# Murmeldyret/cubesat-APDS

Measured on AMD Instinct MI355X. Metric: frames/sec (detect+match+homography) 4k×4k tile vs 1M-desc DB; Mmatches/sec, higher is better.
Workload: dtype fp4 e2m1 operands / f32 accumulate = exact integer Hamming (match), f32 (AKAZE), f64 (homography solve)

## Files before the change

### cubesat-apds_amd/csrc/hamming_mfma.hip

```cpp
#include <atomic>
#include <memory>

#include "config.h"
#include "kernels.h"

namespace apds {

typedef int hm_v8i __attribute__((ext_vector_type(8)));
typedef float hm_f32x4 __attribute__((ext_vector_type(4)));

#ifndef APDS_HM_WAVES
#define APDS_HM_WAVES 8
#endif
static constexpr int HM_WAVES = APDS_HM_WAVES;
static constexpr int HM_TM = 16 * HM_WAVES;
#ifndef APDS_HM_WPE
#define APDS_HM_WPE 4
#endif
#ifndef APDS_HM_NC
#define APDS_HM_NC 3
#endif
static constexpr int HM_NC = APDS_HM_NC;
static constexpr int HM_Q = HM_WAVES * 16 * HM_NC;
static constexpr int HM_UNIT_SCALE = 0x7F7F7F7F;
static constexpr uint64_t HM_EMPTY = ~0ull;
static constexpr int HM_BIAS = 1024;

__device__ __forceinline__ uint32_t hm_spread8(uint32_t b, uint32_t nib) {
    uint32_t t = b & 0xFFu;
    t = (t | (t << 12)) & 0x000F000Fu;
    t = (t | (t << 6)) & 0x03030303u;
    t = (t | (t << 3)) & 0x11111111u;
    return t * nib;
}

__global__ __launch_bounds__(256) void hm_expand_rows_kernel(const uint32_t* __restrict__ rows, long long n, uint32_t nib, int bias, uint4* __restrict__ out,
                                                             float* __restrict__ pc) {
    APDS_RAISE_WAVE_PRIORITY();
    const long long i = (long long)blockIdx.x * 256 + threadIdx.x;
    const uint32_t d = i < n * 16 ? rows[i] : 0u;
    int v = __popc(d);
#pragma unroll
    for (int off = 8; off > 0; off >>= 1) v += __shfl_xor(v, off);
    if (i >= n * 16) return;
    out[i] = make_uint4(hm_spread8(d, nib), hm_spread8(d >> 8, nib), hm_spread8(d >> 16, nib), hm_spread8(d >> 24, nib));
    if ((threadIdx.x & 15) == 0) pc[i >> 4] = (float)(v + bias);
}

__global__ void hm_pad_rows_kernel(uint4* __restrict__ rows, float* __restrict__ pc, long long n, long long n_pad) {
    const long long i = n + (threadIdx.x >> 4);
    if (i >= n_pad) return;
    for (long long r = i; r < n_pad; r += 8) {
        rows[r * 16 + (threadIdx.x & 15)] = make_uint4(0, 0, 0, 0);
        if ((threadIdx.x & 15) == 0) pc[r] = INFINITY;
    }
}

__global__ void hm_thresholds_kernel(const uint64_t* __restrict__ topk, int K, const float* __restrict__ qpc, int nq, uint32_t* __restrict__ thr) {
    const int i = blockIdx.x * blockDim.x + threadIdx.x;
    if (i >= nq) return;
    const uint64_t k2 = topk[(size_t)i * K + K - 1];
    thr[i] = k2 == HM_EMPTY ? 0x7F800000u : __float_as_uint((float)((int)(uint32_t)(k2 >> 32) - (int)qpc[i] + HM_BIAS));
}

struct HmTop2 {
    uint32_t d0, d1;
    uint32_t i0, i1;
};
__device__ __forceinline__ void hm_insert(HmTop2& b, uint32_t d, uint32_t idx) {
    if (d < b.d1) {
        if (d < b.d0) {
            b.d1 = b.d0;
            b.i1 = b.i0;
            b.d0 = d;
            b.i0 = idx;
        } else {
            b.d1 = d;
            b.i1 = idx;
        }
    }
}

template <int PRIO, bool THR>
__global__ __launch_bounds__(64 * HM_WAVES) __attribute__((amdgpu_waves_per_eu(APDS_HM_WPE, APDS_HM_WPE))) void hamming_mfma_kernel(const uint4* __restrict__ train_fp4, const float* __restrict__ tpc, int n_train,
                                                           const uint4* __restrict__ query_fp4, const float* __restrict__ qpc, int nq, int tiles_per_split,
                                                           int q_tiles, int splits, uint32_t index_base, const uint32_t* __restrict__ thr,
                                                           uint64_t* __restrict__ out) {
    extern __shared__ __attribute__((aligned(128))) unsigned char hm_lds[];
    constexpr int TILE_BYTES = HM_TM * 256;
    const int tid = threadIdx.x, lane = tid & 63, wave = tid >> 6;
    int split, qtile;
    if ((splits & 7) == 0) {
        const int xcd = blockIdx.x & 7, j = blockIdx.x >> 3;
        split = xcd + 8 * (j / q_tiles);
        qtile = j % q_tiles;
    } else {
        split = blockIdx.x / q_tiles;
        qtile = blockIdx.x % q_tiles;
    }
    const int q0 = qtile * HM_Q + wave * 16 * HM_NC;
    const int n_tiles = (n_train + HM_TM - 1) / HM_TM;
    const int tile_begin = split * tiles_per_split, tile_end = min(n_tiles, tile_begin + tiles_per_split);
    const int col = lane & 15, kq = lane >> 4;

    uint4 B[HM_NC][4];
    float qq[HM_NC];
#pragma unroll
    for (int c = 0; c < HM_NC; c++) {
        const int qi = min(q0 + 16 * c + col, nq - 1);
#pragma unroll
        for (int s = 0; s < 4; s++) B[c][s] = query_fp4[(size_t)qi * 16 + 4 * s + kq];
        qq[c] = qpc[qi];
    }
    HmTop2 best[HM_NC];
#pragma unroll
    for (int c = 0; c < HM_NC; c++) {
        best[c].d0 = best[c].d1 = THR ? thr[min(q0 + 16 * c + col, nq - 1)] : 0x7F800000u;
        best[c].i0 = best[c].i1 = 0xFFFFFFFFu;
    }

    if (tile_begin < tile_end) {
        int soff[4];
#pragma unroll
        for (int i = 0; i < 4; i++) {
            const int r = 16 * wave + 4 * i + (lane >> 4);
            soff[i] = r * 256 + (((lane & 15) ^ (r & 15)) << 4);
        }
        auto stage = [&](int tile, int buf) {
            const unsigned char* tbase = reinterpret_cast<const unsigned char*>(train_fp4) + (size_t)tile * TILE_BYTES;
#pragma unroll
            for (int i = 0; i < 4; i++)
                __builtin_amdgcn_global_load_lds((const __attribute__((address_space(1))) void*)(tbase + soff[i]),
                                                 (__attribute__((address_space(3))) void*)(hm_lds + buf * TILE_BYTES + (16 * wave + 4 * i) * 256), 16, 0, 0);
            if (wave < HM_TM / 64)
                __builtin_amdgcn_global_load_lds((const __attribute__((address_space(1))) void*)(tpc + (size_t)tile * HM_TM + 64 * wave + lane),
                                                 (__attribute__((address_space(3))) void*)(hm_lds + 2 * TILE_BYTES + buf * (HM_TM * 4) + 256 * wave), 4, 0, 0);
        };
        int aoff[4];
#pragma unroll
        for (int s = 0; s < 4; s++) aoff[s] = col * 256 + (((4 * s + kq) ^ col) << 4);
        const int noff = 2 * TILE_BYTES + 16 * kq;

        hm_f32x4 acc[HM_NC];
        auto rank = [&](const hm_f32x4 (&a)[HM_NC], uint32_t row0) {
            bool hit[HM_NC];
#pragma unroll
            for (int c = 0; c < HM_NC; c++) {
                const uint32_t mn = min(min(__float_as_uint(a[c][0]), __float_as_uint(a[c][1])), min(__float_as_uint(a[c][2]), __float_as_uint(a[c][3])));
                hit[c] = mn < best[c].d1;
            }
#pragma unroll
            for (int c = 0; c < HM_NC; c++)
                if (__any(hit[c])) {
#pragma unroll
                    for (int j = 0; j < 4; j++) hm_insert(best[c], __float_as_uint(a[c][j]), row0 + j);
                }
        };

        stage(tile_begin, 0);
        __syncthreads();
        for (int tile = tile_begin; tile < tile_end; tile++) {
            const int buf = (tile - tile_begin) & 1;
            if (tile + 1 < tile_end) stage(tile + 1, buf ^ 1);
            const unsigned char* T = hm_lds + buf * TILE_BYTES;
            const unsigned char* Nn = hm_lds + noff + buf * (HM_TM * 4);
#pragma unroll
            for (int rb = 0; rb < HM_TM / 16; rb++) {
                const hm_f32x4 init = *reinterpret_cast<const hm_f32x4*>(Nn + rb * 64);
                uint4 a[4];
#pragma unroll
                for (int s = 0; s < 4; s++) a[s] = *reinterpret_cast<const uint4*>(T + rb * 4096 + aoff[s]);
                auto steps = [&](int s_lo, int s_hi) {
#pragma unroll
                    for (int s = s_lo; s < s_hi; s++) {
                        const hm_v8i A = {(int)a[s].x, (int)a[s].y, (int)a[s].z, (int)a[s].w, 0, 0, 0, 0};
#pragma unroll
                        for (int c = 0; c < HM_NC; c++) {
                            const hm_v8i Bv = {(int)B[c][s].x, (int)B[c][s].y, (int)B[c][s].z, (int)B[c][s].w, 0, 0, 0, 0};
                            acc[c] = __builtin_amdgcn_mfma_scale_f32_16x16x128_f8f6f4(A, Bv, s == 0 ? init : acc[c], 4, 4, 0, HM_UNIT_SCALE, 0, HM_UNIT_SCALE);
                        }
                    }
                };
                if (PRIO) __builtin_amdgcn_s_setprio(PRIO);
                steps(0, 4);
                if (PRIO) __builtin_amdgcn_s_setprio(0);
                rank(acc, (uint32_t)(tile * HM_TM + rb * 16 + 4 * kq) + index_base);
            }
            __syncthreads();
        }
    }
#pragma unroll
    for (int c = 0; c < HM_NC; c++) {
        HmTop2 b = best[c];
#pragma unroll
        for (int off = 16; off < 64; off <<= 1) {
            const uint32_t od0 = (uint32_t)__shfl_xor((int)b.d0, off), od1 = (uint32_t)__shfl_xor((int)b.d1, off);
            const uint32_t oi0 = (uint32_t)__shfl_xor((int)b.i0, off), oi1 = (uint32_t)__shfl_xor((int)b.i1, off);
            HmTop2 m = b;
            auto ins = [&](uint32_t d, uint32_t i) {
                if (i == 0xFFFFFFFFu) return;
                if (d < m.d0 || (d == m.d0 && i < m.i0)) {
                    m.d1 = m.d0;
                    m.i1 = m.i0;
                    m.d0 = d;
                    m.i0 = i;
                } else if ((d < m.d1 || (d == m.d1 && i < m.i1)) && i != m.i0) {
                    m.d1 = d;
                    m.i1 = i;
                }
            };
            ins(od0, oi0);
            ins(od1, oi1);
            b = m;
        }
        const int qi = q0 + 16 * c + col;
        if (kq == 0 && qi < nq) {
            uint64_t* o = out + ((size_t)split * nq + qi) * 2;
            o[0] = b.i0 == 0xFFFFFFFFu ? HM_EMPTY : ((uint64_t)(uint32_t)((int)(qq[c] + __uint_as_float(b.d0)) - HM_BIAS) << 32) | b.i0;
            o[1] = b.i1 == 0xFFFFFFFFu ? HM_EMPTY : ((uint64_t)(uint32_t)((int)(qq[c] + __uint_as_float(b.d1)) - HM_BIAS) << 32) | b.i1;
        }
    }
}

template <int K>
struct HmTopK {
    uint32_t d[K];
    uint32_t i[K];
};
template <int K>
__device__ __forceinline__ void hm_insert_k(HmTopK<K>& b, uint32_t d, uint32_t idx) {
#pragma unroll
    for (int j = K - 1; j > 0; j--) {
        const bool shift = d < b.d[j - 1], here = d < b.d[j];
        b.i[j] = shift ? b.i[j - 1] : (here ? idx : b.i[j]);
        b.d[j] = shift ? b.d[j - 1] : (here ? d : b.d[j]);
    }
    const bool first = d < b.d[0];
    b.i[0] = first ? idx : b.i[0];
    b.d[0] = first ? d : b.d[0];
}
__device__ __forceinline__ uint64_t hm_shfl_xor_u64(uint64_t v, int off) {
    return ((uint64_t)(uint32_t)__shfl_xor((int)(uint32_t)(v >> 32), off) << 32) | (uint32_t)__shfl_xor((int)(uint32_t)v, off);
}

#ifndef APDS_HM_NC_K4
#define APDS_HM_NC_K4 2
#endif
#ifndef APDS_HM_NC_K8
#define APDS_HM_NC_K8 2
#endif
template <int K>
struct HmShape {
    static constexpr int NC = K <= 4 ? APDS_HM_NC_K4 : APDS_HM_NC_K8;
    static constexpr int Q = HM_WAVES * 16 * NC;
};

template <int K, int NC, int PRIO, bool THR>
__global__ __launch_bounds__(64 * HM_WAVES) __attribute__((amdgpu_waves_per_eu(APDS_HM_WPE, APDS_HM_WPE))) void hamming_mfma_topk_kernel(
    const uint4* __restrict__ train_fp4, const float* __restrict__ tpc, int n_train, const uint4* __restrict__ query_fp4, const float* __restrict__ qpc, int nq,
    int tiles_per_split, int q_tiles, int splits, uint32_t index_base, const uint32_t* __restrict__ thr, uint64_t* __restrict__ out) {
    extern __shared__ __attribute__((aligned(128))) unsigned char hm_lds[];
    constexpr int TILE_BYTES = HM_TM * 256;
    const int tid = threadIdx.x, lane = tid & 63, wave = tid >> 6;
    int split, qtile;
    if ((splits & 7) == 0) {
        const int xcd = blockIdx.x & 7, j = blockIdx.x >> 3;
        split = xcd + 8 * (j / q_tiles);
        qtile = j % q_tiles;
    } else {
        split = blockIdx.x / q_tiles;
        qtile = blockIdx.x % q_tiles;
    }
    const int q0 = qtile * (HM_WAVES * 16 * NC) + wave * 16 * NC;
    const int n_tiles = (n_train + HM_TM - 1) / HM_TM;
    const int tile_begin = split * tiles_per_split, tile_end = min(n_tiles, tile_begin + tiles_per_split);
    const int col = lane & 15, kq = lane >> 4;

    uint4 B[NC][4];
    float qq[NC];
#pragma unroll
    for (int c = 0; c < NC; c++) {
        const int qi = min(q0 + 16 * c + col, nq - 1);
#pragma unroll
        for (int s = 0; s < 4; s++) B[c][s] = query_fp4[(size_t)qi * 16 + 4 * s + kq];
        qq[c] = qpc[qi];
    }
    HmTopK<K> best[NC];
#pragma unroll
    for (int c = 0; c < NC; c++) {
        const uint32_t start = THR ? thr[min(q0 + 16 * c + col, nq - 1)] : 0x7F800000u;
#pragma unroll
        for (int j = 0; j < K; j++) best[c].d[j] = start, best[c].i[j] = 0xFFFFFFFFu;
    }

    if (tile_begin < tile_end) {
        int soff[4];
#pragma unroll
        for (int i = 0; i < 4; i++) {
            const int r = 16 * wave + 4 * i + (lane >> 4);
            soff[i] = r * 256 + (((lane & 15) ^ (r & 15)) << 4);
        }
        auto stage = [&](int tile, int buf) {
            const unsigned char* tbase = reinterpret_cast<const unsigned char*>(train_fp4) + (size_t)tile * TILE_BYTES;
#pragma unroll
            for (int i = 0; i < 4; i++)
                __builtin_amdgcn_global_load_lds((const __attribute__((address_space(1))) void*)(tbase + soff[i]),
                                                 (__attribute__((address_space(3))) void*)(hm_lds + buf * TILE_BYTES + (16 * wave + 4 * i) * 256), 16, 0, 0);
            if (wave < HM_TM / 64)
                __builtin_amdgcn_global_load_lds((const __attribute__((address_space(1))) void*)(tpc + (size_t)tile * HM_TM + 64 * wave + lane),
                                                 (__attribute__((address_space(3))) void*)(hm_lds + 2 * TILE_BYTES + buf * (HM_TM * 4) + 256 * wave), 4, 0, 0);
        };
        int aoff[4];
#pragma unroll
        for (int s = 0; s < 4; s++) aoff[s] = col * 256 + (((4 * s + kq) ^ col) << 4);
        const int noff = 2 * TILE_BYTES + 16 * kq;

        hm_f32x4 acc[NC];
        auto rank = [&](const hm_f32x4 (&a)[NC], uint32_t row0) {
            bool hit[NC];
#pragma unroll
            for (int c = 0; c < NC; c++) {
                const uint32_t mn = min(min(__float_as_uint(a[c][0]), __float_as_uint(a[c][1])), min(__float_as_uint(a[c][2]), __float_as_uint(a[c][3])));
                hit[c] = mn < best[c].d[K - 1];
            }
#pragma unroll
            for (int c = 0; c < NC; c++)
                if (__any(hit[c])) {
#pragma unroll
                    for (int j = 0; j < 4; j++) {
                        const uint32_t v = __float_as_uint(a[c][j]);
                        if (__any(v < best[c].d[K - 1])) hm_insert_k<K>(best[c], v, row0 + j);
                    }
                }
        };

        stage(tile_begin, 0);
        __syncthreads();
        for (int tile = tile_begin; tile < tile_end; tile++) {
            const int buf = (tile - tile_begin) & 1;
            if (tile + 1 < tile_end) stage(tile + 1, buf ^ 1);
            const unsigned char* T = hm_lds + buf * TILE_BYTES;
            const unsigned char* Nn = hm_lds + noff + buf * (HM_TM * 4);
#pragma unroll
            for (int rb = 0; rb < HM_TM / 16; rb++) {
                const hm_f32x4 init = *reinterpret_cast<const hm_f32x4*>(Nn + rb * 64);
                uint4 a[4];
#pragma unroll
                for (int s = 0; s < 4; s++) a[s] = *reinterpret_cast<const uint4*>(T + rb * 4096 + aoff[s]);
                if (PRIO) __builtin_amdgcn_s_setprio(PRIO);
#pragma unroll
                for (int s = 0; s < 4; s++) {
                    const hm_v8i A = {(int)a[s].x, (int)a[s].y, (int)a[s].z, (int)a[s].w, 0, 0, 0, 0};
#pragma unroll
                    for (int c = 0; c < NC; c++) {
                        const hm_v8i Bv = {(int)B[c][s].x, (int)B[c][s].y, (int)B[c][s].z, (int)B[c][s].w, 0, 0, 0, 0};
                        acc[c] = __builtin_amdgcn_mfma_scale_f32_16x16x128_f8f6f4(A, Bv, s == 0 ? init : acc[c], 4, 4, 0, HM_UNIT_SCALE, 0, HM_UNIT_SCALE);
                    }
                }
                if (PRIO) __builtin_amdgcn_s_setprio(0);
                rank(acc, (uint32_t)(tile * HM_TM + rb * 16 + 4 * kq) + index_base);
            }
            __syncthreads();
        }
    }
#pragma unroll
    for (int c = 0; c < NC; c++) {
        uint64_t key[K];
#pragma unroll
        for (int j = 0; j < K; j++) key[j] = ((uint64_t)best[c].d[j] << 32) | best[c].i[j];
#pragma unroll
        for (int off = 16; off < 64; off <<= 1) {
            uint64_t other[K];
#pragma unroll
            for (int j = 0; j < K; j++) other[j] = hm_shfl_xor_u64(key[j], off);
#pragma unroll
            for (int j = 0; j < K; j++) key[j] = min(key[j], other[K - 1 - j]);
#pragma unroll
            for (int step = K / 2; step > 0; step >>= 1)
#pragma unroll
                for (int j = 0; j < K; j++)
                    if ((j & step) == 0) {
                        const uint64_t lo = min(key[j], key[j + step]), hi = max(key[j], key[j + step]);
                        key[j] = lo;
                        key[j + step] = hi;
                    }
        }
        const int qi = q0 + 16 * c + col;
        if (kq == 0 && qi < nq) {
            uint64_t* o = out + ((size_t)split * nq + qi) * K;
#pragma unroll
            for (int j = 0; j < K; j++) {
                const uint32_t d = (uint32_t)(key[j] >> 32), i = (uint32_t)key[j];
                o[j] = i == 0xFFFFFFFFu ? HM_EMPTY : ((uint64_t)(uint32_t)((int)(qq[c] + __uint_as_float(d)) - HM_BIAS) << 32) | i;
            }
        }
    }
}

static int hm_list_len(int k) { return k <= 2 ? 2 : (k <= 4 ? 4 : 8); }
static int hm_queries_per_block(int K) { return K <= 2 ? HM_Q : (K <= 4 ? HmShape<4>::Q : HmShape<8>::Q); }

HmPlan hm_plan(int nq, long long nt, int K) {
    HmPlan p;
    p.q_tiles = ceil_div(nq, hm_queries_per_block(K));
    const int t_tiles = (int)ceil_div(nt, (long long)HM_TM);
    constexpr int SLOTS = 256 * (16 / HM_WAVES);
    constexpr int OVERHEAD = 4;
    const int max_splits = (int)std::max<long long>(1, std::min<long long>(std::min(t_tiles, 128), (32ll << 20) / std::max(K, 2) / std::max(nq, 1)));
    long long best_cost = -1;
    p.splits = 1;
    for (int sp = 1; sp <= max_splits; sp++) {
        const long long rounds = ceil_div((long long)p.q_tiles * sp, (long long)SLOTS);
        const long long cost = rounds * (ceil_div(t_tiles, sp) + OVERHEAD);
        if (best_cost < 0 || cost < best_cost) best_cost = cost, p.splits = sp;
    }
    if (config().match_mfma_xcd && t_tiles >= 64) {
        long long best8 = -1;
        int sp8 = 0;
        for (int sp = 8; sp <= std::min(max_splits, 32); sp += 8) {
            const long long rounds = ceil_div((long long)p.q_tiles * sp, (long long)SLOTS);
            const long long cost = rounds * (ceil_div(t_tiles, sp) + OVERHEAD);
            if (best8 < 0 || cost < best8) best8 = cost, sp8 = sp;
        }
        if (sp8 && best8 * 100 <= best_cost * 105) {
            p.splits = sp8;
            p.tiles_per_split = ceil_div(t_tiles, p.splits);
            return p;
        }
    }
    if (config().match_mfma_splits > 0) p.splits = std::min(t_tiles, config().match_mfma_splits);
    p.tiles_per_split = ceil_div(t_tiles, p.splits);
    p.splits = ceil_div(t_tiles, p.tiles_per_split);
    return p;
}

void hm_expand_device(const void* rows64, long long n, bool query, void* out_fp4, float* pc, hipStream_t s) {
    if (n <= 0) return;
    hipLaunchKernelGGL(hm_expand_rows_kernel, dim3((unsigned)ceil_div(n * 16, 256)), dim3(256), 0, s, static_cast<const uint32_t*>(rows64), n, query ? 0xCu : 0x2u,
                       query ? 0 : HM_BIAS, static_cast<uint4*>(out_fp4), pc);
    if (!query && hm_padded_rows(n) > n)
        hipLaunchKernelGGL(hm_pad_rows_kernel, dim3(1), dim3(128), 0, s, static_cast<uint4*>(out_fp4), pc, n, hm_padded_rows(n));
}
long long hm_padded_rows(long long n) { return ceil_div(n, (long long)HM_TM) * HM_TM; }
long long hm_sample_rows(long long nt) {
    const long long cap = config().match_mfma_sample;
    return (cap > 0 && nt >= 65536) ? std::min<long long>(cap, nt / 16 / HM_TM * HM_TM) / HM_TM * HM_TM : 0;
}

template <int K>
static void hm_scan_k_launch(const void* q_fp4, const float* qpc, int nq, const void* t_fp4, const float* tpc, long long nt, const HmPlan& p, uint32_t index_base,
                             uint64_t* parts, hipStream_t s, const uint32_t* thr, size_t lds) {
    constexpr int NC = HmShape<K>::NC;
    static std::atomic<bool> opted_dev[64];
    std::atomic<bool>& opted = opted_dev[ctx().device & 63];
    if (!opted.load()) {
        auto opt = [&](auto kernel) { HIP_CHECK(hipFuncSetAttribute(reinterpret_cast<const void*>(kernel), hipFuncAttributeMaxDynamicSharedMemorySize, 160 * 1024)); };
        opt(&hamming_mfma_topk_kernel<K, NC, 0, false>), opt(&hamming_mfma_topk_kernel<K, NC, 2, false>);
        opt(&hamming_mfma_topk_kernel<K, NC, 0, true>), opt(&hamming_mfma_topk_kernel<K, NC, 2, true>);
        opted.store(true);
    }
    auto go = [&](auto kernel) {
        hipLaunchKernelGGL(kernel, dim3((unsigned)p.q_tiles * p.splits), dim3(64 * HM_WAVES), lds, s, static_cast<const uint4*>(t_fp4), tpc, (int)nt,
                           static_cast<const uint4*>(q_fp4), qpc, nq, p.tiles_per_split, p.q_tiles, p.splits, index_base, thr, parts);
    };
    const bool prio = config().match_mfma_prio > 0;
    if (thr) prio ? go(&hamming_mfma_topk_kernel<K, NC, 2, true>) : go(&hamming_mfma_topk_kernel<K, NC, 0, true>);
    else prio ? go(&hamming_mfma_topk_kernel<K, NC, 2, false>) : go(&hamming_mfma_topk_kernel<K, NC, 0, false>);
}

void hm_scan_device(const void* q_fp4, const float* qpc, int nq, const void* t_fp4, const float* tpc, long long nt, const HmPlan& p, uint32_t index_base,
                    uint64_t* parts, hipStream_t s, const uint32_t* thr, bool timed, int K) {
    const size_t lds = (size_t)2 * HM_TM * 256 + 2 * HM_TM * sizeof(float) + (size_t)std::max(0, config().match_mfma_lds_pad);
    if (K > 2) {
        APDS_REQUIRE(K == 4 || K == 8, APDS_ERR_ASSERT, "the matrix-core matcher keeps lists of 2, 4 or 8");
        std::unique_ptr<KernelTimer> timer, timer_k;
        if (timed) timer.reset(new KernelTimer("hamming_topk", s)), timer_k.reset(new KernelTimer("hamming_topk_mfma_k", s));
        if (K == 4) hm_scan_k_launch<4>(q_fp4, qpc, nq, t_fp4, tpc, nt, p, index_base, parts, s, thr, lds);
        else hm_scan_k_launch<8>(q_fp4, qpc, nq, t_fp4, tpc, nt, p, index_base, parts, s, thr, lds);
        return;
    }
    static std::atomic<bool> opted_dev[64];
    std::atomic<bool>& opted = opted_dev[ctx().device & 63];
    if (!opted.load()) {
        auto opt = [&](auto kernel) { HIP_CHECK(hipFuncSetAttribute(reinterpret_cast<const void*>(kernel), hipFuncAttributeMaxDynamicSharedMemorySize, 160 * 1024)); };
        opt(&hamming_mfma_kernel<0, false>), opt(&hamming_mfma_kernel<1, false>), opt(&hamming_mfma_kernel<2, false>), opt(&hamming_mfma_kernel<3, false>);
        opt(&hamming_mfma_kernel<0, true>), opt(&hamming_mfma_kernel<1, true>), opt(&hamming_mfma_kernel<2, true>), opt(&hamming_mfma_kernel<3, true>);
        opted.store(true);
    }
    std::unique_ptr<KernelTimer> timer;
    if (timed) timer.reset(new KernelTimer("hamming_topk", s));
    auto go = [&](auto kernel) {
        hipLaunchKernelGGL(kernel, dim3((unsigned)p.q_tiles * p.splits), dim3(64 * HM_WAVES), lds, s, static_cast<const uint4*>(t_fp4), tpc, (int)nt,
                           static_cast<const uint4*>(q_fp4), qpc, nq, p.tiles_per_split, p.q_tiles, p.splits, index_base, thr, parts);
    };
    const int prio = std::max(0, std::min(3, config().match_mfma_prio));
    if (thr) {
        switch (prio) {
            case 0: go(&hamming_mfma_kernel<0, true>); break;
            case 1: go(&hamming_mfma_kernel<1, true>); break;
            case 2: go(&hamming_mfma_kernel<2, true>); break;
            default: go(&hamming_mfma_kernel<3, true>); break;
        }
    } else {
        switch (prio) {
            case 0: go(&hamming_mfma_kernel<0, false>); break;
            case 1: go(&hamming_mfma_kernel<1, false>); break;
            case 2: go(&hamming_mfma_kernel<2, false>); break;
            default: go(&hamming_mfma_kernel<3, false>); break;
        }
    }
}

void* hm_train_create(const void* rows64, long long n, hipStream_t s) {
    APDS_REQUIRE(rows64 && n > 0 && n < (1ll << 31), APDS_ERR_ASSERT, "an expanded train set needs rows");
    HmTrain* t = new HmTrain();
    t->device = ctx().device;
    t->src = rows64;
    t->n = n;
    if (hipMalloc(&t->rows, (size_t)hm_padded_rows(n) * 256) != hipSuccess || hipMalloc(reinterpret_cast<void**>(&t->pc), (size_t)hm_padded_rows(n) * 4) != hipSuccess) {
        (void)hipGetLastError();
        if (t->rows) (void)hipFree(t->rows);
        delete t;
        fail(APDS_ERR_NOMEM, "no device memory for the expanded train rows");
    }
    hm_expand_device(rows64, n, false, t->rows, t->pc, s);
    HIP_CHECK(hipStreamSynchronize(s));
    return t;
}
void hm_train_destroy(void* h) {
    HmTrain* t = static_cast<HmTrain*>(h);
    if (!t) return;
    int previous = -1;
    if (hipGetDevice(&previous) != hipSuccess) previous = -1;
    (void)hipSetDevice(t->device);
    (void)hipDeviceSynchronize();
    if (t->rows) (void)hipFree(t->rows);
    if (t->pc) (void)hipFree(t->pc);
    delete t;
    if (previous >= 0) (void)hipSetDevice(previous);
}

static void hm_topk_expanded(const void* q, int nq, const void* t4, const float* tp, long long nt, uint32_t index_base, int k, uint64_t* out, hipStream_t s) {
    ThreadCtx& c = ctx();
    void* q4 = c.alloc((size_t)nq * 256);
    float* qp = c.alloc_n<float>(nq);
    {
        KernelTimer timer("hamming_topk_sample", s);
        hm_expand_device(q, nq, true, q4, qp, s);
    }
    const long long sample = hm_sample_rows(nt);
    const int K = hm_list_len(k);
    uint64_t* topk = k == K ? out : c.alloc_n<uint64_t>((size_t)nq * K);
    if (sample) {
        const HmPlan pa = hm_plan(nq, sample, K), pb = hm_plan(nq, nt - sample, K);
        uint64_t* parts_a = c.alloc_n<uint64_t>((size_t)pa.splits * nq * K);
        uint64_t* parts_b = c.alloc_n<uint64_t>((size_t)(pb.splits + 1) * nq * K);
        uint64_t* topk_a = parts_b + (size_t)pb.splits * nq * K;
        uint32_t* thr = c.alloc_n<uint32_t>(nq);
        {
            KernelTimer timer("hamming_topk_sample", s);
            hm_scan_device(q4, qp, nq, t4, tp, sample, pa, index_base, parts_a, s, nullptr, false, K);
            if (pa.splits > 1) merge_topk_device(parts_a, pa.splits, nq, K, topk_a, s);
            else HIP_CHECK(hipMemcpyAsync(topk_a, parts_a, (size_t)nq * K * 8, hipMemcpyDeviceToDevice, s));
            hipLaunchKernelGGL(hm_thresholds_kernel, dim3(ceil_div(nq, 256)), dim3(256), 0, s, (const uint64_t*)topk_a, K, (const float*)qp, nq, thr);
        }
        hm_scan_device(q4, qp, nq, static_cast<const char*>(t4) + (size_t)sample * 256, tp + sample, nt - sample, pb, index_base + (uint32_t)sample, parts_b, s, thr,
                       true, K);
        merge_topk_device(parts_b, pb.splits + 1, nq, K, topk, s);
    } else {
        const HmPlan p = hm_plan(nq, nt, K);
        uint64_t* parts = p.splits == 1 ? topk : c.alloc_n<uint64_t>((size_t)p.splits * nq * K);
        hm_scan_device(q4, qp, nq, t4, tp, nt, p, index_base, parts, s, nullptr, true, K);
        if (p.splits > 1) merge_topk_device(parts, p.splits, nq, K, topk, s);
    }
    if (k != K) take_first_columns_device(topk, nq, K, k, out, s);
    HIP_CHECK(hipGetLastError());
}

void hamming_mfma_topk_device(const void* q, int nq, const void* t, long long nt, uint32_t index_base, int k, uint64_t* out, hipStream_t s) {
    APDS_REQUIRE(k >= 1 && k <= 8, APDS_ERR_ASSERT, "the matrix-core matcher serves 1 <= k <= 8");
    APDS_REQUIRE(nq > 0 && nt > 0 && nt < (1ll << 31), APDS_ERR_ASSERT, "the matrix-core matcher needs queries and train rows");
    ThreadCtx& c = ctx();
    void* t4 = c.alloc((size_t)hm_padded_rows(nt) * 256);
    float* tp = c.alloc_n<float>(hm_padded_rows(nt));
    {
        KernelTimer timer("hamming_topk_sample", s);
        hm_expand_device(t, nt, false, t4, tp, s);
    }
    hm_topk_expanded(q, nq, t4, tp, nt, index_base, k, out, s);
}

void hamming_mfma_topk_train_device(const void* q, int nq, const void* train, uint32_t index_base, int k, uint64_t* out, hipStream_t s) {
    const HmTrain* t = static_cast<const HmTrain*>(train);
    APDS_REQUIRE(t && k >= 1 && k <= 8 && nq > 0, APDS_ERR_ASSERT, "the matrix-core matcher needs an expanded train set, queries and 1 <= k <= 8");
    hm_topk_expanded(q, nq, t->rows, t->pc, t->n, index_base, k, out, s);
}

}
```

Measured before the change: 142.5.

## Software-pipeline LDS reads and hand-issue global_load_lds in shared Hamming tile scan

Result: faster. 151.6 (median of 6 runs) (+6.4%).

```diff
diff --git a/cubesat-apds_amd/csrc/hamming_mfma.hip b/cubesat-apds_amd/csrc/hamming_mfma.hip
--- a/cubesat-apds_amd/csrc/hamming_mfma.hip
+++ b/cubesat-apds_amd/csrc/hamming_mfma.hip
@@ -8,6 +8,7 @@
 
 typedef int hm_v8i __attribute__((ext_vector_type(8)));
 typedef float hm_f32x4 __attribute__((ext_vector_type(4)));
+typedef uint32_t hm_u32x4 __attribute__((ext_vector_type(4)));
 
 #ifndef APDS_HM_WAVES
 #define APDS_HM_WAVES 8
@@ -81,13 +82,118 @@
     }
 }
 
+__device__ __forceinline__ void hm_dma_rows(const unsigned char* tile_base, const int (&voff)[4], uint32_t lds_dst) {
+    uint32_t keep;
+    asm volatile(
+        "s_mov_b32 %0, m0\n\t"
+        "s_mov_b32 m0, %6\n\t"
+        "s_nop 0\n\t"
+        "global_load_lds_dwordx4 %1, %5\n\t"
+        "global_load_lds_dwordx4 %2, %5 offset:1024\n\t"
+        "global_load_lds_dwordx4 %3, %5 offset:2048\n\t"
+        "global_load_lds_dwordx4 %4, %5 offset:3072\n\t"
+        "s_mov_b32 m0, %0"
+        : "=&s"(keep)
+        : "v"(voff[0]), "v"(voff[1]), "v"(voff[2]), "v"(voff[3]), "s"(tile_base), "s"(lds_dst)
+        : "memory");
+}
+__device__ __forceinline__ void hm_dma_popcounts(const float* src, int voff, uint32_t lds_dst) {
+    uint32_t keep;
+    asm volatile(
+        "s_mov_b32 %0, m0\n\t"
+        "s_mov_b32 m0, %3\n\t"
+        "s_nop 0\n\t"
+        "global_load_lds_dword %1, %2\n\t"
+        "s_mov_b32 m0, %0"
+        : "=&s"(keep)
+        : "v"(voff), "s"(src), "s"(lds_dst)
+        : "memory");
+}
+__device__ __forceinline__ void hm_dma_wait() { asm volatile("s_waitcnt vmcnt(0)" ::: "memory"); }
+template <class T>
+__device__ __forceinline__ void hm_settle(T& v) { asm volatile("" : "+v"(v)); }
+
+template <int NC, int PRIO, class Rank>
+__device__ __forceinline__ void hm_scan_tiles(const uint4* __restrict__ train_fp4, const float* __restrict__ tpc, int tile_begin, int tile_end,
+                                              uint4 (&B)[NC][4], uint32_t index_base, Rank&& rank) {
+    extern __shared__ __attribute__((aligned(128))) unsigned char hm_lds[];
+    constexpr int TILE_BYTES = HM_TM * 256;
+    const int lane = threadIdx.x & 63, wave = __builtin_amdgcn_readfirstlane(threadIdx.x >> 6);
+    const int col = lane & 15, kq = lane >> 4;
+    const uint32_t lds0 = (uint32_t)(__SIZE_TYPE__)(__attribute__((address_space(3))) unsigned char*)hm_lds;
+    int voff[4];
+#pragma unroll
+    for (int i = 0; i < 4; i++) {
+        const int r = 16 * wave + 4 * i + (lane >> 4);
+        voff[i] = r * 256 + (((lane & 15) ^ (r & 15)) << 4) - 1024 * i;
+    }
+    auto stage = [&](int tile, int buf) {
+        hm_dma_rows(reinterpret_cast<const unsigned char*>(train_fp4) + (size_t)tile * TILE_BYTES, voff, lds0 + buf * TILE_BYTES + 16 * wave * 256);
+        if (wave < HM_TM / 64) hm_dma_popcounts(tpc + (size_t)tile * HM_TM + 64 * wave, 4 * lane, lds0 + 2 * TILE_BYTES + buf * (HM_TM * 4) + 256 * wave);
+    };
+    typedef const __attribute__((address_space(3))) hm_u32x4* lds_u4;
+    typedef const __attribute__((address_space(3))) hm_f32x4* lds_f4;
+    uint32_t ra[4], rn = lds0 + 2 * TILE_BYTES + 16 * kq;
+#pragma unroll
+    for (int s = 0; s < 4; s++) ra[s] = lds0 + col * 256 + (((4 * s + kq) ^ col) << 4);
+
+    hm_u32x4 a[4];
+    hm_f32x4 init;
+    auto read_block = [&](int rb) {
+#pragma unroll
+        for (int s = 0; s < 4; s++) a[s] = *(lds_u4)(__SIZE_TYPE__)(ra[s] + rb * 4096);
+        init = *(lds_f4)(__SIZE_TYPE__)(rn + rb * 64);
+    };
+
+#pragma unroll
+    for (int c = 0; c < NC; c++)
+#pragma unroll
+        for (int s = 0; s < 4; s++) hm_settle(B[c][s].x), hm_settle(B[c][s].y), hm_settle(B[c][s].z), hm_settle(B[c][s].w);
+    hm_dma_wait();
+    stage(tile_begin, 0);
+    hm_dma_wait();
+    __syncthreads();
+    read_block(0);
+    hm_f32x4 acc[NC];
+    for (int tile = tile_begin; tile < tile_end; tile++) {
+        const int buf = (tile - tile_begin) & 1;
+        if (tile + 1 < tile_end) stage(tile + 1, buf ^ 1);
+#pragma unroll
+        for (int rb = 0; rb < HM_TM / 16; rb++) {
+            if (PRIO) __builtin_amdgcn_s_setprio(PRIO);
+#pragma unroll
+            for (int s = 0; s < 4; s++) {
+                const hm_v8i A = {(int)a[s].x, (int)a[s].y, (int)a[s].z, (int)a[s].w, 0, 0, 0, 0};
+#pragma unroll
+                for (int c = 0; c < NC; c++) {
+                    const hm_v8i Bv = {(int)B[c][s].x, (int)B[c][s].y, (int)B[c][s].z, (int)B[c][s].w, 0, 0, 0, 0};
+                    acc[c] = __builtin_amdgcn_mfma_scale_f32_16x16x128_f8f6f4(A, Bv, s == 0 ? init : acc[c], 4, 4, 0, HM_UNIT_SCALE, 0, HM_UNIT_SCALE);
+                }
+            }
+            if (PRIO) __builtin_amdgcn_s_setprio(0);
+            if (rb + 1 < HM_TM / 16) {
+                read_block(rb + 1);
+            } else {
+                hm_dma_wait();
+                __syncthreads();
+#pragma unroll
+                for (int s = 0; s < 4; s++) ra[s] += buf ? -TILE_BYTES : TILE_BYTES;
+                rn += buf ? -HM_TM * 4 : HM_TM * 4;
+                read_block(0);
+            }
+#pragma unroll
+            for (int c = 0; c < NC; c++) hm_settle(acc[c]);
+            __builtin_amdgcn_sched_barrier(0);
+            rank(acc, (uint32_t)(tile * HM_TM + rb * 16 + 4 * kq) + index_base);
+        }
+    }
+}
+
 template <int PRIO, bool THR>
 __global__ __launch_bounds__(64 * HM_WAVES) __attribute__((amdgpu_waves_per_eu(APDS_HM_WPE, APDS_HM_WPE))) void hamming_mfma_kernel(const uint4* __restrict__ train_fp4, const float* __restrict__ tpc, int n_train,
                                                            const uint4* __restrict__ query_fp4, const float* __restrict__ qpc, int nq, int tiles_per_split,
                                                            int q_tiles, int splits, uint32_t index_base, const uint32_t* __restrict__ thr,
                                                            uint64_t* __restrict__ out) {
-    extern __shared__ __attribute__((aligned(128))) unsigned char hm_lds[];
-    constexpr int TILE_BYTES = HM_TM * 256;
     const int tid = threadIdx.x, lane = tid & 63, wave = tid >> 6;
     int split, qtile;
     if ((splits & 7) == 0) {
@@ -115,34 +221,14 @@
     HmTop2 best[HM_NC];
 #pragma unroll
     for (int c = 0; c < HM_NC; c++) {
-        best[c].d0 = best[c].d1 = THR ? thr[min(q0 + 16 * c + col, nq - 1)] : 0x7F800000u;
+        best[c].d0 = THR ? thr[min(q0 + 16 * c + col, nq - 1)] : 0x7F800000u;
+        hm_settle(best[c].d0), hm_settle(qq[c]);
+        best[c].d1 = best[c].d0;
         best[c].i0 = best[c].i1 = 0xFFFFFFFFu;
     }
 
     if (tile_begin < tile_end) {
-        int soff[4];
-#pragma unroll
-        for (int i = 0; i < 4; i++) {
-            const int r = 16 * wave + 4 * i + (lane >> 4);
-            soff[i] = r * 256 + (((lane & 15) ^ (r & 15)) << 4);
-        }
-        auto stage = [&](int tile, int buf) {
-            const unsigned char* tbase = reinterpret_cast<const unsigned char*>(train_fp4) + (size_t)tile * TILE_BYTES;
-#pragma unroll
-            for (int i = 0; i < 4; i++)
-                __builtin_amdgcn_global_load_lds((const __attribute__((address_space(1))) void*)(tbase + soff[i]),
-                                                 (__attribute__((address_space(3))) void*)(hm_lds + buf * TILE_BYTES + (16 * wave + 4 * i) * 256), 16, 0, 0);
-            if (wave < HM_TM / 64)
-                __builtin_amdgcn_global_load_lds((const __attribute__((address_space(1))) void*)(tpc + (size_t)tile * HM_TM + 64 * wave + lane),
-                                                 (__attribute__((address_space(3))) void*)(hm_lds + 2 * TILE_BYTES + buf * (HM_TM * 4) + 256 * wave), 4, 0, 0);
-        };
-        int aoff[4];
-#pragma unroll
-        for (int s = 0; s < 4; s++) aoff[s] = col * 256 + (((4 * s + kq) ^ col) << 4);
-        const int noff = 2 * TILE_BYTES + 16 * kq;
-
-        hm_f32x4 acc[HM_NC];
-        auto rank = [&](const hm_f32x4 (&a)[HM_NC], uint32_t row0) {
+        hm_scan_tiles<HM_NC, PRIO>(train_fp4, tpc, tile_begin, tile_end, B, index_base, [&](const hm_f32x4 (&a)[HM_NC], uint32_t row0) {
             bool hit[HM_NC];
 #pragma unroll
             for (int c = 0; c < HM_NC; c++) {
@@ -155,39 +241,7 @@
 #pragma unroll
                     for (int j = 0; j < 4; j++) hm_insert(best[c], __float_as_uint(a[c][j]), row0 + j);
                 }
-        };
-
-        stage(tile_begin, 0);
-        __syncthreads();
-        for (int tile = tile_begin; tile < tile_end; tile++) {
-            const int buf = (tile - tile_begin) & 1;
-            if (tile + 1 < tile_end) stage(tile + 1, buf ^ 1);
-            const unsigned char* T = hm_lds + buf * TILE_BYTES;
-            const unsigned char* Nn = hm_lds + noff + buf * (HM_TM * 4);
-#pragma unroll
-            for (int rb = 0; rb < HM_TM / 16; rb++) {
-                const hm_f32x4 init = *reinterpret_cast<const hm_f32x4*>(Nn + rb * 64);
-                uint4 a[4];
-#pragma unroll
-                for (int s = 0; s < 4; s++) a[s] = *reinterpret_cast<const uint4*>(T + rb * 4096 + aoff[s]);
-                auto steps = [&](int s_lo, int s_hi) {
-#pragma unroll
-                    for (int s = s_lo; s < s_hi; s++) {
-                        const hm_v8i A = {(int)a[s].x, (int)a[s].y, (int)a[s].z, (int)a[s].w, 0, 0, 0, 0};
-#pragma unroll
-                        for (int c = 0; c < HM_NC; c++) {
-                            const hm_v8i Bv = {(int)B[c][s].x, (int)B[c][s].y, (int)B[c][s].z, (int)B[c][s].w, 0, 0, 0, 0};
-                            acc[c] = __builtin_amdgcn_mfma_scale_f32_16x16x128_f8f6f4(A, Bv, s == 0 ? init : acc[c], 4, 4, 0, HM_UNIT_SCALE, 0, HM_UNIT_SCALE);
-                        }
-                    }
-                };
-                if (PRIO) __builtin_amdgcn_s_setprio(PRIO);
-                steps(0, 4);
-                if (PRIO) __builtin_amdgcn_s_setprio(0);
-                rank(acc, (uint32_t)(tile * HM_TM + rb * 16 + 4 * kq) + index_base);
-            }
-            __syncthreads();
-        }
+        });
     }
 #pragma unroll
     for (int c = 0; c < HM_NC; c++) {
@@ -259,8 +313,6 @@
 __global__ __launch_bounds__(64 * HM_WAVES) __attribute__((amdgpu_waves_per_eu(APDS_HM_WPE, APDS_HM_WPE))) void hamming_mfma_topk_kernel(
     const uint4* __restrict__ train_fp4, const float* __restrict__ tpc, int n_train, const uint4* __restrict__ query_fp4, const float* __restrict__ qpc, int nq,
     int tiles_per_split, int q_tiles, int splits, uint32_t index_base, const uint32_t* __restrict__ thr, uint64_t* __restrict__ out) {
-    extern __shared__ __attribute__((aligned(128))) unsigned char hm_lds[];
-    constexpr int TILE_BYTES = HM_TM * 256;
     const int tid = threadIdx.x, lane = tid & 63, wave = tid >> 6;
     int split, qtile;
     if ((splits & 7) == 0) {
@@ -288,35 +340,14 @@
     HmTopK<K> best[NC];
 #pragma unroll
     for (int c = 0; c < NC; c++) {
-        const uint32_t start = THR ? thr[min(q0 + 16 * c + col, nq - 1)] : 0x7F800000u;
+        uint32_t start = THR ? thr[min(q0 + 16 * c + col, nq - 1)] : 0x7F800000u;
+        hm_settle(start), hm_settle(qq[c]);
 #pragma unroll
         for (int j = 0; j < K; j++) best[c].d[j] = start, best[c].i[j] = 0xFFFFFFFFu;
     }
 
     if (tile_begin < tile_end) {
-        int soff[4];
-#pragma unroll
-        for (int i = 0; i < 4; i++) {
-            const int r = 16 * wave + 4 * i + (lane >> 4);
-            soff[i] = r * 256 + (((lane & 15) ^ (r & 15)) << 4);
-        }
-        auto stage = [&](int tile, int buf) {
-            const unsigned char* tbase = reinterpret_cast<const unsigned char*>(train_fp4) + (size_t)tile * TILE_BYTES;
-#pragma unroll
-            for (int i = 0; i < 4; i++)
-                __builtin_amdgcn_global_load_lds((const __attribute__((address_space(1))) void*)(tbase + soff[i]),
-                                                 (__attribute__((address_space(3))) void*)(hm_lds + buf * TILE_BYTES + (16 * wave + 4 * i) * 256), 16, 0, 0);
-            if (wave < HM_TM / 64)
-                __builtin_amdgcn_global_load_lds((const __attribute__((address_space(1))) void*)(tpc + (size_t)tile * HM_TM + 64 * wave + lane),
-                                                 (__attribute__((address_space(3))) void*)(hm_lds + 2 * TILE_BYTES + buf * (HM_TM * 4) + 256 * wave), 4, 0, 0);
-        };
-        int aoff[4];
-#pragma unroll
-        for (int s = 0; s < 4; s++) aoff[s] = col * 256 + (((4 * s + kq) ^ col) << 4);
-        const int noff = 2 * TILE_BYTES + 16 * kq;
-
-        hm_f32x4 acc[NC];
-        auto rank = [&](const hm_f32x4 (&a)[NC], uint32_t row0) {
+        hm_scan_tiles<NC, PRIO>(train_fp4, tpc, tile_begin, tile_end, B, index_base, [&](const hm_f32x4 (&a)[NC], uint32_t row0) {
             bool hit[NC];
 #pragma unroll
             for (int c = 0; c < NC; c++) {
@@ -332,36 +363,7 @@
                         if (__any(v < best[c].d[K - 1])) hm_insert_k<K>(best[c], v, row0 + j);
                     }
                 }
-        };
-
-        stage(tile_begin, 0);
-        __syncthreads();
-        for (int tile = tile_begin; tile < tile_end; tile++) {
-            const int buf = (tile - tile_begin) & 1;
-            if (tile + 1 < tile_end) stage(tile + 1, buf ^ 1);
-            const unsigned char* T = hm_lds + buf * TILE_BYTES;
-            const unsigned char* Nn = hm_lds + noff + buf * (HM_TM * 4);
-#pragma unroll
-            for (int rb = 0; rb < HM_TM / 16; rb++) {
-                const hm_f32x4 init = *reinterpret_cast<const hm_f32x4*>(Nn + rb * 64);
-                uint4 a[4];
-#pragma unroll
-                for (int s = 0; s < 4; s++) a[s] = *reinterpret_cast<const uint4*>(T + rb * 4096 + aoff[s]);
-                if (PRIO) __builtin_amdgcn_s_setprio(PRIO);
-#pragma unroll
-                for (int s = 0; s < 4; s++) {
-                    const hm_v8i A = {(int)a[s].x, (int)a[s].y, (int)a[s].z, (int)a[s].w, 0, 0, 0, 0};
-#pragma unroll
-                    for (int c = 0; c < NC; c++) {
-                        const hm_v8i Bv = {(int)B[c][s].x, (int)B[c][s].y, (int)B[c][s].z, (int)B[c][s].w, 0, 0, 0, 0};
-                        acc[c] = __builtin_amdgcn_mfma_scale_f32_16x16x128_f8f6f4(A, Bv, s == 0 ? init : acc[c], 4, 4, 0, HM_UNIT_SCALE, 0, HM_UNIT_SCALE);
-                    }
-                }
-                if (PRIO) __builtin_amdgcn_s_setprio(0);
-                rank(acc, (uint32_t)(tile * HM_TM + rb * 16 + 4 * kq) + index_base);
-            }
-            __syncthreads();
-        }
+        });
     }
 #pragma unroll
     for (int c = 0; c < NC; c++) {
```
